# arnab39/equiadapt

Hardware: AMD Instinct MI355X
Metric: canonicalize+invert images/sec (224x224 C8) (higher is better)
Workload: dtype f32 (resampling / FFT / accumulation in fp32; the network's channel contraction as 2xfp16 split of every fp32 operand (within one fp32 ulp), 3 exact products, fp32 accumulate -- closer to fp64 than the fp32 matrix instruction, see step_ms_by_gemm_form); 1 GPU; configs[1]: 224x224x3 synthetic, C8, GroupEquivariantImageCanonicalization + ESCNNEquivariantNetwork in e2cnn's LAYER SHAPES (32 fields x 8 = 256 ch, k5, 3 layers, crop 0.8, resize 96) with this repository's own filter-bank parameterisation (bilinear-rotated banks; e2cnn's steerable basis is not restated -- e2cnn-trained weights enter via load_exported_dense), forward, then invert_canonicalization; batch_per_gpu=256, global_batch=256, parallelism=dp1 (no collective in the forward path)

## Files before the change

equiadapt_amd/_lib.py:

```python
import ctypes
import os
import subprocess
import threading

_HERE = os.path.dirname(os.path.abspath(__file__))
ROOT = os.path.dirname(_HERE)
CSRC = os.path.join(_HERE, "csrc")
SO_PATH = os.environ.get("EQA_LIB") or os.path.join(CSRC, "libeqa_hip.so")
SOURCES = [os.path.join(CSRC, f) for f in ("group_action.hip", "crop_resize.hip", "nearest_action.hip", "pooling.hip", "batchnorm.hip", "winograd.hip", "lift_conv.hip", "lift_conv_wide.hip", "lift_wgrad.hip", "pointcloud.hip", "vnsmall_train.hip", "vnsmall_tail.hip", "fftconv.hip", "fft_filter.hip", "lift_fft.hip", "cgemm3m.hip", "cgemm3m_bf16.hip", "smallconv.hip", "planegemm.hip", "convnet_train.hip")]
HEADERS = [os.path.join(CSRC, "eqa_common.hpp"), os.path.join(CSRC, "vn_common.hpp"), os.path.join(CSRC, "fft48.inc"), os.path.join(CSRC, "fft_common.inc"), os.path.join(CSRC, "cgemm3m_common.inc")]
INCLUDE = os.path.join(ROOT, "include")

ABI_VERSION = 3

_c_f = ctypes.POINTER(ctypes.c_float)
_c_i = ctypes.POINTER(ctypes.c_int32)
_vp = ctypes.c_void_p
_int = ctypes.c_int

SIGNATURES = {
    "eqa_abi_version": (_int, []),
    "eqa_set_option": (_int, [_int, _int]),
    "eqa_get_option": (_int, [_int]),
    "eqa_fold_edge_pad_workspace_bytes": (ctypes.c_int64, [_int] * 4),
    "eqa_fold_edge_pad": (_int, [_vp, _vp, _vp, _int, _int, _int, _int, _vp]),
    "eqa_canon_transform_fwd": (_int, [_vp, _vp, _vp, _vp, _vp] + [_int] * 6 + [_vp]),
    "eqa_invert_action_fwd": (_int, [_vp, _vp, _vp, _vp, _vp, _vp] + [_int] * 6 + [_vp]),
    "eqa_group_action_pair": (_int, [_vp] * 4 + [_int, _int] + [_vp] * 5 + [_int, _int, _vp] + [_int] * 4 + [_vp]),
    "eqa_orbit_expand_fwd": (_int, [_vp, _vp, _vp, _vp] + [_int] * 5 + [_vp]),
    "eqa_group_action_fwd": (_int, [_vp, _vp, _vp, _vp, _vp, _vp] + [_int] * 12 + [_vp]),
    "eqa_group_action_fwd_hint": (_int, [_vp, _vp, _vp, _vp, _vp, _vp] + [_int] * 13 + [_vp]),
    "eqa_crop_resize_aa": (_int, [_vp] * 6 + [_int] * 9 + [_vp]),
    "eqa_mask_action_nearest": (_int, [_vp] * 5 + [_int] * 4 + [_vp]),
    "eqa_mask_action_nearest_planes": (_int, [_vp] * 5 + [_int] * 4 + [_vp]),
    "eqa_boxes_action": (_int, [_vp] * 5 + [_int, ctypes.c_float, _int, _vp]),
    "eqa_image_action_nearest": (_int, [_vp] * 5 + [_int] * 10 + [_vp]),
    "eqa_group_action_bwd_tiles": (_int, [_int, _int]),
    "eqa_group_action_bwd": (_int, [_vp] * 8 + [_int] * 12 + [_vp]),
    "eqa_group_action_bwd_theta": (_int, [_vp] * 8 + [_int] * 12 + [_vp]),
    "eqa_group_pool_workspace_bytes": (ctypes.c_int64, [_int] * 4),
    "eqa_group_pool_argmax": (_int, [_vp, _vp, _vp, _vp] + [_int] * 4 + [_vp]),
    "eqa_window_sums": (_int, [_vp, _vp, _vp, _int, _vp] + [_int] * 5 + [_vp]),
    "eqa_bn_partial_blocks": (ctypes.c_int64, [ctypes.c_int64]),
    "eqa_bn_stats_nhwc": (_int, [_vp, _vp, ctypes.c_int64, _int, _vp]),
    "eqa_bn_relu_dropout_nhwc": (_int, [_vp, _vp, _vp, _vp, ctypes.c_int64, _int, ctypes.c_float, ctypes.c_uint32, _vp]),
    "eqa_bn_bwd_reduce_nhwc": (_int, [_vp] * 5 + [ctypes.c_float, _vp, ctypes.c_int64, _int, _vp, _vp, ctypes.c_uint32, _vp]),
    "eqa_bn_bwd_apply_nhwc": (_int, [_vp] * 8 + [ctypes.c_float, _vp, ctypes.c_int64, _int, _vp, _vp, ctypes.c_uint32, _vp]),
# ... 264 lines not shown
```

equiadapt_amd/csrc/crop_resize.hip:

```cpp
#include "eqa_common.hpp"

namespace {

constexpr int kAaBand = 8;
#ifndef EQA_AA_WIDE_MIN_K
#define EQA_AA_WIDE_MIN_K 8
#endif
constexpr int kAaMaxK = 20;

__global__ __launch_bounds__(kThreads) void crop_resize_aa_kernel(const float* __restrict__ x, float* __restrict__ y,
                                                                 const float* __restrict__ wx, const int32_t* __restrict__ x0,
                                                                 const float* __restrict__ wy, const int32_t* __restrict__ y0,
                                                                 int H, int W, int OH, int OW, int K, int max_rows) {
  extern __shared__ __attribute__((aligned(16))) float aa_tmp[];
  const int plane = blockIdx.y;
  const int r0 = blockIdx.x * kAaBand, r1 = min(r0 + kAaBand, OH);
  const int ybeg = y0[r0];
  const int yend = min(y0[r1 - 1] + K, H);
  const int nrows = min(yend - ybeg, max_rows);
  const float* src = x + (size_t)plane * H * W;
  const int rows_par = kThreads / OW;
  if (rows_par >= 1) {
    const int ox = threadIdx.x % OW, rsub = threadIdx.x / OW;
    if (rsub < rows_par) {
      const int xs = x0[ox];
      float wv[EQA_AA_WIDE_MIN_K];
      int xo[EQA_AA_WIDE_MIN_K];
#pragma unroll
// ... 14 lines not shown
      }
    }
  } else {
    for (int idx = threadIdx.x; idx < nrows * OW; idx += kThreads) {
      const int ry = idx / OW, ox = idx - ry * OW;
      const float* row = src + (size_t)(ybeg + ry) * W;
      const int xs = x0[ox];
      float acc = 0.0f;
#pragma unroll
      for (int j = 0; j < EQA_AA_WIDE_MIN_K; ++j)
        if (j < K) acc += wx[ox * K + j] * row[min(xs + j, W - 1)];
      aa_tmp[ry * OW + ox] = acc;
    }
  }
  __syncthreads();
  float* dst = y + (size_t)plane * OH * OW;
  for (int idx = threadIdx.x; idx < (r1 - r0) * OW; idx += kThreads) {
    const int r = idx / OW, ox = idx - r * OW;
    const int oy = r0 + r;

    const int ys = y0[oy] - ybeg;
    float acc = 0.0f;
#pragma unroll
    for (int j = 0; j < EQA_AA_WIDE_MIN_K; ++j)
      if (j < K) acc += wy[oy * K + j] * aa_tmp[min(ys + j, nrows - 1) * OW + ox];
    dst[(size_t)oy * OW + ox] = acc;
  }
}


template <int K, int BAND, int NL>
__global__ __launch_bounds__(kThreads, (NL > 5 && K > 5) ? 2 : 4) void crop_resize_aa_staged_kernel(
    const float* __restrict__ x, float* __restrict__ y,
                                                                        const float* __restrict__ wx, const int32_t* __restrict__ x0,
                                                                        const float* __restrict__ wy, const int32_t* __restrict__ y0,
                                                                        int planes, int H, int W, int OH, int OW, int cap_rows,
                                                                        int xb, int xl) {
  extern __shared__ __attribute__((aligned(16))) float aa_tmp[];
  float* rows = aa_tmp;
  float* tmp = aa_tmp + (size_t)cap_rows * xl;
  float* tabw = tmp + (size_t)cap_rows * OW;
  int* taby = reinterpret_cast<int*>(tabw + BAND * K);
  const int r0 = blockIdx.y * BAND, r1 = min(r0 + BAND, OH);
  const int nband = r1 - r0;
  const int plane0 = (int)(blockIdx.z * kXcd + blockIdx.x), plane_step = (int)(gridDim.z * kXcd);
  const int rows_par = kThreads / OW;
  const int ox = rows_par >= 1 ? threadIdx.x % OW : 0, rsub = rows_par >= 1 ? threadIdx.x / OW : 0;
  const int xs_g = x0[ox];
  float wv[K];
  int xo[K];
#pragma unroll
  for (int j = 0; j < K; ++j) {
    wv[j] = wx[ox * K + j];
    xo[j] = min(xs_g - xb + j, xl - 1);
  }
  if ((int)threadIdx.x < nband * K) tabw[threadIdx.x] = wy[r0 * K + threadIdx.x];
  const int ybeg = y0[r0];
  if ((int)threadIdx.x < nband) taby[threadIdx.x] = y0[r0 + threadIdx.x] - ybeg;
  const int yend = min(y0[r1 - 1] + K, H);
  const int nrows = min(yend - ybeg, cap_rows);
  const int nq = xl >> 2;
  const int tq = threadIdx.x & 63, tr = threadIdx.x >> 6;
  const bool prefetch = nq <= 64 && nrows <= 4 * NL;
  const size_t plane_sz = (size_t)H * W;
  const float* src0 = x + (size_t)ybeg * W + xb;
  typedef float aa_f4 __attribute__((ext_vector_type(4)));
  aa_f4 v[NL];
#define EQA_AA_PF_LOAD(plane_)                                                                                          \
  do {                                                                                                                  \
    const float* src_ = src0 + (size_t)(plane_) * plane_sz;                                                             \
    _Pragma("unroll") for (int k = 0; k < NL; ++k)                                                           \
      v[k] = *reinterpret_cast<const aa_f4*>(src_ + (size_t)min(tr + 4 * k, nrows - 1) * W + 4 * min(tq, nq - 1));     \
  } while (0)
  __builtin_amdgcn_s_waitcnt(0x0070);
  if (prefetch && plane0 < planes) EQA_AA_PF_LOAD(plane0);
  for (int plane = plane0; plane < planes; plane += plane_step) {
    if (prefetch) {
      if (tq < nq) {
#pragma unroll
        for (int k = 0; k < NL; ++k)
          if (tr + 4 * k < nrows) *reinterpret_cast<aa_f4*>(rows + (tr + 4 * k) * xl + 4 * tq) = v[k];
      }
      if (plane + plane_step < planes) EQA_AA_PF_LOAD(plane + plane_step);
    } else {
      const float* src = src0 + (size_t)plane * plane_sz;
      for (int q = tq; q < nq; q += 64)
        for (int rb = tr; rb < nrows; rb += 4) *reinterpret_cast<aa_f4*>(rows + rb * xl + 4 * q) = *reinterpret_cast<const aa_f4*>(src + (size_t)rb * W + 4 * q);
    }
    __syncthreads();
    if (rows_par >= 1) {
      if (rsub < rows_par) {
        for (int ry0 = rsub; ry0 < nrows; ry0 += 4 * rows_par) {
          float acc[4] = {0.0f, 0.0f, 0.0f, 0.0f};
#pragma unroll
          for (int u = 0; u < 4; ++u) {
            const float* row = rows + min(ry0 + u * rows_par, nrows - 1) * xl;
#pragma unroll
            for (int j = 0; j < K; ++j)
// ... 6 lines not shown
      }
    } else {
      for (int idx = threadIdx.x; idx < nrows * OW; idx += kThreads) {
        const int ry = idx / OW, oxx = idx - ry * OW;
        const float* row = rows + ry * xl;
        const int xs = x0[oxx] - xb;
        float acc = 0.0f;
#pragma unroll
        for (int j = 0; j < K; ++j)
          acc += wx[oxx * K + j] * row[min(xs + j, xl - 1)];
        tmp[ry * OW + oxx] = acc;
      }
    }
    __syncthreads();
    float* dst = y + (size_t)plane * OH * OW;
    for (int idx = threadIdx.x; idx < nband * OW; idx += kThreads) {
      const int r = idx / OW, oxx = idx - r * OW;
      const int ys = taby[r];
      float acc = 0.0f;
#pragma unroll
      for (int j = 0; j < K; ++j)
        acc += tabw[r * K + j] * tmp[min(ys + j, nrows - 1) * OW + oxx];
      dst[(size_t)(r0 + r) * OW + oxx] = acc;
    }
    __syncthreads();
  }
#undef EQA_AA_PF_LOAD
}

__global__ __launch_bounds__(kThreads) void crop_resize_aa_wide_kernel(const float* __restrict__ x, float* __restrict__ y,
                                                                      const float* __restrict__ wx, const int32_t* __restrict__ x0,
                                                                      const float* __restrict__ wy, const int32_t* __restrict__ y0,
                                                                      int H, int W, int OH, int OW, int K, int max_rows, int xbeg,
                                                                      int xlen, int pad_shift, int row_stride, int rpi) {
  extern __shared__ __attribute__((aligned(16))) float aa_tmp[];
  float* rowbuf = aa_tmp + (size_t)max_rows * OW;
  const int plane = blockIdx.y;
  const int r0 = blockIdx.x * kAaBand, r1 = min(r0 + kAaBand, OH);
  const int ybeg = y0[r0];
  const int yend = min(y0[r1 - 1] + K, H);
  const int nrows = min(yend - ybeg, max_rows);
  const float* src = x + (size_t)plane * H * W;
  auto pos = [&](int e) { return pad_shift ? e + (e >> pad_shift) : e; };
  const bool fixed_col = (kThreads % OW) == 0 && K <= kAaMaxK;
  const bool vec_stage = rpi <= 8 && (xlen & 3) == 0 && (xbeg & 3) == 0 && (W & 3) == 0 && ((((uintptr_t)src) & 15) == 0);
  const int ox_fixed = threadIdx.x % OW;
  const int xs_fixed = x0[ox_fixed] - xbeg;
  float wreg[kAaMaxK];
#pragma unroll
// ... 52 lines not shown
          if (j < K) acc += wreg[j] * row[pos(min(xs_fixed + j, xlen - 1))];
        aa_tmp[(ry0 + rr) * OW + ox_fixed] = acc;
      }
    } else {
      for (int idx = threadIdx.x; idx < nr * OW; idx += kThreads) {
        const int rr = idx / OW, ox = idx - rr * OW;
        const float* row = rowbuf + rr * row_stride;
        const int xs = x0[ox] - xbeg;
        float acc = 0.0f;
        for (int j = 0; j < K; ++j) acc += wx[ox * K + j] * row[pos(min(xs + j, xlen - 1))];
        aa_tmp[(ry0 + rr) * OW + ox] = acc;
      }
    }
    __syncthreads();
  }
  float* dst = y + (size_t)plane * OH * OW;
  for (int idx = threadIdx.x; idx < (r1 - r0) * OW; idx += kThreads) {
    const int r = idx / OW, ox = idx - r * OW;
    const int oy = r0 + r;
    const int ys = y0[oy] - ybeg;
    float acc = 0.0f;
    for (int j = 0; j < K; ++j) acc += wy[oy * K + j] * aa_tmp[min(ys + j, nrows - 1) * OW + ox];
    dst[(size_t)oy * OW + ox] = acc;
  }
}

constexpr int kAaStreamRows = 8;
__global__ __launch_bounds__(kThreads) void crop_resize_aa_stream_kernel(const float* __restrict__ x, float* __restrict__ y,
                                                                        const float* __restrict__ wx, const int32_t* __restrict__ x0,
                                                                        const float* __restrict__ wy, const int32_t* __restrict__ y0,
                                                                        int H, int W, int OH, int OW, int K, int xbeg, int xlen,
                                                                        int pad_shift, int row_stride) {
  extern __shared__ __attribute__((aligned(16))) float aa_rows[];
  const int plane = blockIdx.y;
  const int r0 = blockIdx.x * kAaBand, nr_out = min(kAaBand, OH - r0);
  int ys[kAaBand];
#pragma unroll
  for (int r = 0; r < kAaBand; ++r) ys[r] = y0[r0 + min(r, nr_out - 1)];
  const int ybeg = ys[0];
  const int span = ys[kAaBand - 1] + K - ybeg;
  const float* src = x + (size_t)plane * H * W + xbeg;
  const int e = 4 * (int)threadIdx.x;
  const int e_ld = min(e, xlen - 4);
  auto pos = [&](int i) { return pad_shift ? i + (i >> pad_shift) : i; };
  float4 acc[kAaBand];
#pragma unroll
  for (int r = 0; r < kAaBand; ++r) acc[r] = make_float4(0.f, 0.f, 0.f, 0.f);
// ... 19 lines not shown
        acc[r].x += w * v[q].x; acc[r].y += w * v[q].y; acc[r].z += w * v[q].z; acc[r].w += w * v[q].w;
      }
    }
  };
  static_assert(kAaStreamRows == 8 && kAaBand == 8, "one weight per lane: 8 rows of a trip x 8 output rows = 64 lanes");
  float4 va[kAaStreamRows], vb[kAaStreamRows];
  float wa, wb = 0.0f;
  load8(va, 0);
  wa = wload(0);
  for (int yc = 0; yc < span; yc += 2 * kAaStreamRows) {
    if (yc + kAaStreamRows < span) { load8(vb, yc + kAaStreamRows); wb = wload(yc + kAaStreamRows); }
    add8(va, wa);
    if (yc + 2 * kAaStreamRows < span) { load8(va, yc + 2 * kAaStreamRows); wa = wload(yc + 2 * kAaStreamRows); }
    if (yc + kAaStreamRows < span) add8(vb, wb);
  }
  float* dst = y + (size_t)plane * OH * OW;
#pragma unroll
  for (int half = 0; half < 2; ++half) {
    if (e < xlen) {
#pragma unroll
      for (int rr = 0; rr < kAaBand / 2; ++rr) {
        float* lrow = aa_rows + rr * row_stride;
        const float4 v = acc[half * (kAaBand / 2) + rr];
        lrow[pos(e)] = v.x; lrow[pos(e + 1)] = v.y; lrow[pos(e + 2)] = v.z; lrow[pos(e + 3)] = v.w;
      }
    }
    __syncthreads();
    for (int idx = threadIdx.x; idx < (kAaBand / 2) * OW; idx += kThreads) {
      const int rr = idx / OW, ox = idx - rr * OW;
      const int r = half * (kAaBand / 2) + rr;
      if (r < nr_out) {
        const float* row = aa_rows + rr * row_stride;
        const int xs = x0[ox] - xbeg;
        float a = 0.0f;
        for (int j = 0; j < K; ++j) a += wx[ox * K + j] * row[pos(min(xs + j, xlen - 1))];
        dst[(size_t)(r0 + r) * OW + ox] = a;
      }
    }
    __syncthreads();
  }
}

}

extern "C" {

int eqa_crop_resize_aa(const float* x, float* y, const float* wx, const int32_t* x0, const float* wy, const int32_t* y0,
                       int planes, int H, int W, int OH, int OW, int K, int max_rows, int x_begin, int x_span, void* stream) {
  if (!x || !y || !wx || !x0 || !wy || !y0 || planes < 0 || H <= 0 || W <= 0 || OH <= 0 || OW <= 0 || K <= 0 || max_rows <= 0)
    return EQA_ERR_INVALID_ARG;
  const size_t lds = (size_t)max_rows * OW * sizeof(float);
  if (lds > 96 * 1024 || planes > 65535) return EQA_ERR_UNSUPPORTED;
  if (planes == 0) return EQA_OK;
  const dim3 grid((OH + kAaBand - 1) / kAaBand, planes);
  if (K > EQA_AA_WIDE_MIN_K && x_span > 0 && x_begin >= 0 && x_begin + x_span <= W) {
    const int stride = (x_span + OW / 2) / OW;
    const int pad_shift = (stride >= 2 && (stride & 1) == 0) ? __builtin_ctz((unsigned)stride) : 0;
    const int row_stride = x_span + (pad_shift ? (x_span >> pad_shift) : 0) + 1;
    const size_t row_bytes = (size_t)row_stride * sizeof(float);
    const int rpi = (int)std::min<size_t>(8, lds + row_bytes <= 96 * 1024 ? (96 * 1024 - lds) / row_bytes : 0);
    const size_t lds2 = lds + (size_t)rpi * row_bytes;
    static const bool stream_off = [] { const char* e = getenv("EQA_AA_STREAM"); return e && e[0] == '0'; }();
    if (!stream_off && x_span <= 4 * kThreads && (x_span & 3) == 0 && (x_begin & 3) == 0 && (W & 3) == 0 && (((uintptr_t)x) & 15) == 0 &&
        (size_t)(kAaBand / 2) * row_bytes <= 64 * 1024) {
      hipLaunchKernelGGL(crop_resize_aa_stream_kernel, grid, dim3(kThreads), (kAaBand / 2) * row_bytes, (hipStream_t)stream, x, y, wx, x0, wy,
                         y0, H, W, OH, OW, K, x_begin, x_span, pad_shift, row_stride);
      return launch_status();
    }
    if (rpi >= 1) {
      hipLaunchKernelGGL(crop_resize_aa_wide_kernel, grid, dim3(kThreads), lds2, (hipStream_t)stream, x, y, wx, x0, wy, y0, H, W, OH,
                         OW, K, max_rows, x_begin, x_span, pad_shift, row_stride, rpi);
      return launch_status();
    }
  }
  static const bool staged_off = [] { const char* e = getenv("EQA_AA_STAGED"); return e && e[0] == '0'; }();
  if (!staged_off && K <= EQA_AA_WIDE_MIN_K && (W & 3) == 0 && (((uintptr_t)x) & 15) == 0 && x_span > 0 && x_begin >= 0 &&
      x_begin + x_span <= W) {
    const int xb = x_begin & ~3, xl = std::min(W, (x_begin + x_span + 3) & ~3) - xb;
    static const int band_env = [] { const char* e = getenv("EQA_AA_BAND"); return e ? atoi(e) : 0; }();
    int band = band_env == 16 ? 16 : (band_env == 8 ? 8 : (OH >= 64 ? 16 : 8));
    auto staged_lds = [&](int bnd) { return ((size_t)(bnd / kAaBand) * max_rows * (xl + OW) + bnd * (EQA_AA_WIDE_MIN_K + 1)) * sizeof(float); };
    if (band == 16 && band_env != 16 && (staged_lds(16) > 64 * 1024 || 16 * K > kThreads)) band = 8;
    const int cap_rows = (band / kAaBand) * max_rows;
    const size_t lds3 = staged_lds(band);
    if (lds3 <= 64 * 1024 && band * K <= kThreads) {
      static const int per_cu = [] { const char* e = getenv("EQA_AA_BLOCKS_PER_CU"); return e ? std::max(1, atoi(e)) : 12; }();
      const int nbands = (OH + band - 1) / band;
      const int groups = std::max(1, (std::min(planes, (256 * per_cu + nbands - 1) / nbands) + kXcd - 1) / kXcd);
      const bool few = cap_rows <= 20;
#define EQA_AA_STAGED(K_)                                                                                                              \
  case K_:                                                                                                                             \
    if (band == 16)                                                                                                                    \
      hipLaunchKernelGGL((crop_resize_aa_staged_kernel<K_, 16, 10>), dim3(kXcd, nbands, groups), dim3(kThreads), lds3, (hipStream_t)stream, x, \
                         y, wx, x0, wy, y0, planes, H, W, OH, OW, cap_rows, xb, xl);                                                   \
    else if (few)                                                                                                                      \
      hipLaunchKernelGGL((crop_resize_aa_staged_kernel<K_, 8, 5>), dim3(kXcd, nbands, groups), dim3(kThreads), lds3, (hipStream_t)stream, x,  \
                         y, wx, x0, wy, y0, planes, H, W, OH, OW, cap_rows, xb, xl);                                                   \
    else                                                                                                                               \
      hipLaunchKernelGGL((crop_resize_aa_staged_kernel<K_, 8, 10>), dim3(kXcd, nbands, groups), dim3(kThreads), lds3, (hipStream_t)stream, x, \
                         y, wx, x0, wy, y0, planes, H, W, OH, OW, cap_rows, xb, xl);                                                   \
    break
      switch (K) {
        EQA_AA_STAGED(1); EQA_AA_STAGED(2); EQA_AA_STAGED(3); EQA_AA_STAGED(4); EQA_AA_STAGED(5); EQA_AA_STAGED(6); EQA_AA_STAGED(7);
        EQA_AA_STAGED(8);
        default: return EQA_ERR_UNSUPPORTED;
      }
#undef EQA_AA_STAGED
      return launch_status();
    }
  }
  hipLaunchKernelGGL(crop_resize_aa_kernel, grid, dim3(kThreads), lds, (hipStream_t)stream, x, y, wx, x0, wy, y0, H, W, OH, OW, K,
                     max_rows);
  return launch_status();
}

}
```

equiadapt_amd/images/canonicalization/discrete_group.py:

```python
import math
from typing import Any, Dict, List, Optional, Tuple, Union

import torch
import torch.nn.functional as F

from equiadapt_amd import ops
from equiadapt_amd.common.basecanonicalization import DiscreteGroupCanonicalization
from equiadapt_amd.images import geometry
from equiadapt_amd.images.transforms import CenterCrop, EdgePad, Resize
from equiadapt_amd.images.utils import (
    canonicalize_masks,
    device_tables,
    canonicalize_boxes,
    flip_boxes,
    flip_masks,
    get_action_on_image_features,
    rotate_boxes,
    rotate_masks,
)



def _get(hyperparams: Any, name: str):
    if isinstance(hyperparams, dict):
# ... 88 lines not shown
        raise NotImplementedError(
            "get_group_activations is not implemented for the DiscreteGroupImageCanonicalization class")

    def get_groupelement(self, x: torch.Tensor) -> Dict[str, torch.Tensor]:
        group_activations = self.get_group_activations(x)
        group_index = self.group_index(group_activations)
        element = self.groupactivations_to_groupelement(group_activations, group_index)
        if not hasattr(self, "canonicalization_info_dict"):
            self.canonicalization_info_dict = {}
        self.canonicalization_info_dict["group_index"] = element.pop("group_index")
        self.canonicalization_info_dict["argmax_index"] = group_index
        self.canonicalization_info_dict["group_element"] = element
        self.canonicalization_info_dict["group_activations"] = group_activations
        return element

    def transformations_before_canonicalization_network_forward(self, x: torch.Tensor) -> torch.Tensor:
        crop, resize = self.crop_canonization, self.resize_canonization
        if (x.is_cuda and x.dtype == torch.float32 and not (torch.is_grad_enabled() and x.requires_grad) and isinstance(resize, Resize)
                and resize.antialias):
            from equiadapt_amd.images.transforms import resized_output_size

            out_hw = resized_output_size(crop.size, resize.size)
            if tuple(out_hw) == tuple(x.shape[-2:]) == tuple(crop.size):
                return x
            key = (tuple(x.shape[-2:]), crop.size, out_hw, str(x.device))
            tabs = self._consts.get(key)
            if tabs is None:
                t = geometry.aa_resize_tables(tuple(x.shape[-2:]), crop.size, out_hw)
                tabs = tuple(v.to(x.device) if isinstance(v, torch.Tensor) else v for v in t)
                self._consts[key] = tabs
            return ops.crop_resize_aa(x, tabs, out_hw)
        return resize(crop(x))


    def canonicalize(self, x: torch.Tensor, targets: Optional[List] = None, **kwargs: Any
                     ) -> Union[torch.Tensor, Tuple[torch.Tensor, List]]:
        self.device = x.device
        element = self.get_groupelement(x)
        gidx = self.canonicalization_info_dict["group_index"]
        reflections = "reflection" in element
        H, W = x.shape[-2:]
        pad = self.pad_size
        theta, flags = device_tables("canonicalize", self.num_rotations, reflections, (H + 2 * pad, W + 2 * pad), x.device)
        x = _CanonTransformFn.apply(x, element["rotation"], element.get("reflection"), gidx, theta, flags, pad,
                                    self.num_rotations)

# ... 44 lines not shown

def _num_group(group_type: str, num_rotations: int) -> int:
    return num_rotations if group_type == "rotation" else 2 * num_rotations


class GroupEquivariantImageCanonicalization(DiscreteGroupImageCanonicalization):

    def __init__(self, canonicalization_network: torch.nn.Module, canonicalization_hyperparams: Any, in_shape: tuple):
        super().__init__(canonicalization_network, canonicalization_hyperparams, in_shape)
        self.group_type = canonicalization_network.group_type
        self.num_rotations = canonicalization_network.num_rotations
        self.num_group = _num_group(self.group_type, self.num_rotations)
        self.group_info_dict = {"num_rotations": self.num_rotations, "num_group": self.num_group}

    def get_group_activations(self, x: torch.Tensor) -> torch.Tensor:
        x = self.transformations_before_canonicalization_network_forward(x)
        return self.canonicalization_network(x)


class OptimizedGroupEquivariantImageCanonicalization(DiscreteGroupImageCanonicalization):

    def __init__(self, canonicalization_network: torch.nn.Module, canonicalization_hyperparams: Any, in_shape: tuple):
        super().__init__(canonicalization_network, canonicalization_hyperparams, in_shape)
        self.group_type = _get(canonicalization_hyperparams, "group_type")
        self.num_rotations = _get(canonicalization_hyperparams, "num_rotations")
        self.artifact_err_wt = _get(canonicalization_hyperparams, "artifact_err_wt")
        self.num_group = _num_group(self.group_type, self.num_rotations)
        self.out_vector_size = canonicalization_network.out_vector_size
        size = _get(canonicalization_hyperparams, "resize_shape")
        self.group_augment_size = int(size)
        gray = self.in_shape[0] == 1
# ... 48 lines not shown
```

equiadapt_amd/images/canonicalization_networks/escnn_networks.py:

```python
import os
from typing import List, Sequence

import torch
import torch.nn as nn
import torch.nn.functional as F

from equiadapt_amd.images.canonicalization_networks.custom_group_equivariant_layers import (
    RotationEquivariantConv,
    RotationEquivariantConvLift,
    RotoReflectionEquivariantConv,
    RotoReflectionEquivariantConvLift,
)
from equiadapt_amd import ops
from equiadapt_amd.common.utils import update_running_stats
from equiadapt_amd.images.canonicalization_networks import fftconv, winograd
from equiadapt_amd.images.canonicalization_networks.pooling import (
    WindowSumsFunction,
    conv_then_group_pool,
    group_pool,
    window_sums_to_activations,
)


class _InnerBatchNorm(nn.BatchNorm3d):
# ... 557 lines not shown
            act = act + 0.0 * torch.stack(hidden_bias).sum().double()
        return act.float()

    def _training_fast_path_ok(self, x: torch.Tensor) -> bool:
        if self._dense or not x.is_cuda or x.dtype != torch.float32 or os.environ.get("EQA_TRAIN_FAST", "1") == "0":
            return False
        if (self.out_channels * self.num_group_elements) % 4 != 0:
            return False
        convs = [m for m in self.eqv_network if hasattr(m, "expanded_weights")]
        if len(convs) < 2 or any(c.stride != 1 or c.padding != 0 for c in convs) or not convs[-1].supports_linear_tail():
            return False
        hw = x.shape[-2] - (self.kernel_size - 1) * (len(convs) - 1)
        k = convs[-1].kernel_size
        return hw >= 2 * k - 1 and x.shape[-1] - (self.kernel_size - 1) * (len(convs) - 1) >= 2 * k - 1 and hw * hw <= 12288

    def forward(self, x: torch.Tensor) -> torch.Tensor:
        if (self.training or torch.is_grad_enabled()) and self._training_fast_path_ok(x):
            return self._forward_training(x)
        if not self.training and not torch.is_grad_enabled() and x.is_cuda and x.dtype == torch.float32:
            convs, norms = self._layers()
            shrink = (self.kernel_size - 1) * (len(convs) - 1)
            oh, ow = x.shape[-2] - shrink, x.shape[-1] - shrink
            if (convs[-1].supports_linear_tail() and 0 < oh and 0 < ow and oh * ow <= 12288
                    and all(n.running_mean is not None and not n.training for n in norms)
                    and all(c.stride == 1 and c.padding == 0 and c.kernel_size == self.kernel_size for c in convs)):
                return self._forward_inference(x)
        if self._dense:
            convs, norms = self._dense
            for i, cv in enumerate(convs):
                x = cv(x)
                if i < len(norms):
                    x = F.relu(norms[i](x))
            fm = x.reshape(x.shape[0], self.out_channels, self.num_group_elements, x.shape[-2], x.shape[-1])
        else:
            fm = self.eqv_network(x)
        return group_pool(fm)
```

equiadapt_amd/images/canonicalization_networks/fftconv.py:

```python
import math
import os
from typing import Optional

import torch

from equiadapt_amd import _lib, ops
from equiadapt_amd.ops import _timed

N, NH, OUT = 48, 25, 44
F = N * (NH - 2) + 2 * NH
ENABLED = os.environ.get("EQA_CONV5_FFT", "1") != "0"
MIN_TILES = int(os.environ.get("EQA_FFT_MIN_TILES", "32"))
TRAIN_FORWARD = os.environ.get("EQA_FFT_TRAIN", "1") != "0"
GEMM = os.environ.get("EQA_FFT_GEMM", "3m")
GEMM_PIECES = os.environ.get("EQA_FFT_GEMM_PIECES", "auto")
AUTO_MIN_CIN = int(os.environ.get("EQA_FFT_GEMM_AUTO_MIN_CIN", "128"))
AUTO_MIN_CIN_H3 = int(os.environ.get("EQA_FFT_GEMM_AUTO_MIN_CIN_H3", "64"))
DCMAX_SLOTS = 256
LAST_FORM = None


def f16_form_takes(cin: int, cout: int) -> bool:
    return cout % 128 == 0 and cin % 32 == 0

# ... 179 lines not shown
    def pieces(self) -> torch.Tensor:
        if self._pieces is None:
            self._pieces = self.split_bf16(self.bank)
        return self._pieces

    def spectra_into(self, V: torch.Tensor, B, st: int) -> Optional[torch.Tensor]:
        lib = _lib.load()
        nimg, C, H, W = self.shape
        dims = (nimg, H + 4, W + 4, C, st)
        px, pV = self.x.data_ptr(), V.data_ptr()
        p_b = self.bias.data_ptr() if self.bias is not None else None
        want_dc = self.relu and isinstance(B, Spectra3M) and gemm_form(B.cin, B.cout, True) == "h3"
        vbound = None
        if LIFT_FFT_FORM == "h2" and px % 16 == 0:
            wh, w_scale = self.pieces_f16()
            xbound = torch.empty(DCMAX_SLOTS, dtype=torch.float32, device=self.device)
            _lib.check(lib.eqa_absmax_slots(px, self.x.numel(), xbound.data_ptr(), st), "eqa_absmax_slots")
            if want_dc:
                vbound = torch.empty(DCMAX_SLOTS, dtype=torch.float32, device=self.device)
            _lib.check(lib.eqa_lift5_fft48k5_input_f16x2(px, wh.data_ptr(), w_scale, xbound.data_ptr(), DCMAX_SLOTS, p_b, int(self.relu), pV,
                                                         vbound.data_ptr() if want_dc else None, *dims), "eqa_lift5_fft48k5_input_f16x2")
        elif LIFT_FFT_FORM == "bf16x3":
            _lib.check(lib.eqa_lift5_fft48k5_input_bf16x3(px, self.pieces().data_ptr(), p_b, int(self.relu), pV, *dims),
                       "eqa_lift5_fft48k5_input_bf16x3")
        elif want_dc:
            vbound = torch.empty(DCMAX_SLOTS, dtype=torch.float32, device=self.device)
            _lib.check(lib.eqa_lift5_fft48k5_input_dcmax(px, self.bank.data_ptr(), p_b, 1, pV, vbound.data_ptr(), *dims),
                       "eqa_lift5_fft48k5_input_dcmax")
        else:
            _lib.check(lib.eqa_lift5_fft48k5_input(px, self.bank.data_ptr(), p_b, int(self.relu), pV, *dims), "eqa_lift5_fft48k5_input")
        return vbound

    def materialize(self) -> torch.Tensor:
        return ops.lift_conv_nhwc(self.x, ops.pack_lift_weights(self.bank), self.bias, self.relu, 5, 5)

# ... 282 lines not shown
```

equiadapt_amd/ops.py:

```python
from typing import Optional, Tuple

import torch

from equiadapt_amd import _lib


MAX_WINDOW_K = 10


def _stream() -> int:
    return _raw_stream(_current_device())


try:
    _raw_stream, _current_device = torch._C._cuda_getCurrentRawStream, torch._C._cuda_getDevice
except AttributeError:
    def _raw_stream(_dev):
        return torch.cuda.current_stream().cuda_stream

    def _current_device():
        return 0


class KernelTimer:
# ... 342 lines not shown
    if pooling not in ("mean", "max"):
        raise ValueError(f"Pooling type {pooling} not supported")
    if three != 3 or params.numel() != (1310 if pooling == "mean" else 1751):
        raise ValueError("vnsmall_canonicalize expects x:(B,3,N) and 1310 (mean) / 1751 (max) packed parameters")
    vec = torch.empty((B, 3, 3), dtype=torch.float32, device=x.device)
    R = torch.empty((B, 3, 3), dtype=torch.float32, device=x.device)
    y = torch.empty_like(x)
    ws = torch.empty((max(lib.eqa_vnsmall_workspace_bytes(B, N), 4) // 4,), dtype=torch.float32, device=x.device)
    with torch.cuda.device(x.device), _timed("vnsmall_fwd"):
        st = lib.eqa_vnsmall_canonicalize(x.data_ptr(), params.data_ptr(), vec.data_ptr(), R.data_ptr(), y.data_ptr(), ws.data_ptr(),
                                          B, N, k, int(pooling == "max"), _stream())
    _lib.check(st, "eqa_vnsmall_canonicalize")
    return vec, R, y


def crop_resize_aa(x: torch.Tensor, tables, out_hw: Tuple[int, int]) -> torch.Tensor:
    lib = _lib.load()
    x = _need(x, "x")
    wx, x0, wy, y0, K, max_rows, x_begin, x_span = tables
    B, C, H, W = x.shape
    y = torch.empty((B, C, out_hw[0], out_hw[1]), dtype=torch.float32, device=x.device)
    with torch.cuda.device(x.device), _timed("crop_resize_aa"):
        st = lib.eqa_crop_resize_aa(x.data_ptr(), y.data_ptr(), wx.data_ptr(), x0.data_ptr(), wy.data_ptr(), y0.data_ptr(),
                                    B * C, H, W, out_hw[0], out_hw[1], K, max_rows, x_begin, x_span, _stream())
    _lib.check(st, "eqa_crop_resize_aa")
    return y


def mask_action_nearest(masks: torch.Tensor, eidx: torch.Tensor, rtheta: torch.Tensor, flags: Optional[torch.Tensor]) -> torch.Tensor:
    lib = _lib.load()
    masks = _need(masks, "masks", torch.uint8)
    eidx = _need(eidx, "eidx", torch.int32)
    rtheta = _need(rtheta, "rtheta")
    flags, p_flags = _opt(flags, "flags", torch.int32)
    n, H, W = masks.shape
# ... 489 lines not shown
```

include/eqa_hip.h:

```cpp
#ifndef EQA_HIP_H
#define EQA_HIP_H

#include <stdint.h>

#ifdef __cplusplus
extern "C" {
#endif

#define EQA_OK 0
#define EQA_ERR_INVALID_ARG (-1)
#define EQA_ERR_LAUNCH (-2)
#define EQA_ERR_UNSUPPORTED (-3)

#define EQA_FLIP_SRC 1
#define EQA_FLIP_DST 2

#define EQA_ABI_VERSION 3
int eqa_abi_version(void);

int eqa_set_option(int key, int value);
int eqa_get_option(int key);

int eqa_canon_transform_fwd(const float* x, float* y, const int32_t* gidx, const float* theta,
                            const int32_t* flags, int num_elements, int B, int C, int H, int W, int pad,
// ... 8 lines not shown
                          const int32_t* chan_map, int G, int Cf, const int32_t* gidx, int num_elements, int B, int H,
                          int W, void* stream);

int eqa_orbit_expand_fwd(const float* x, float* y, const float* theta, const int32_t* flags, int num_elements,
                         int B, int C, int S, int pad, void* stream);

int eqa_group_action_fwd(const float* src, float* dst, const int32_t* gidx, const float* theta,
                         const int32_t* flags, const int32_t* chan_map, int num_elements, int G, int n_out,
                         int B, int C, int H, int W, int pad, int OH, int OW, int top, int left, void* stream);
int eqa_group_action_fwd_hint(const float* src, float* dst, const int32_t* gidx, const float* theta, const int32_t* flags,
                              const int32_t* chan_map, int num_elements, int G, int n_out, int B, int C, int H, int W,
                              int pad, int OH, int OW, int top, int left, int max_window, void* stream);

int eqa_crop_resize_aa(const float* x, float* y, const float* wx, const int32_t* x0, const float* wy, const int32_t* y0,
                       int planes, int H, int W, int OH, int OW, int K, int max_rows, int x_begin, int x_span, void* stream);

int eqa_mask_action_nearest(const uint8_t* m, uint8_t* out, const int32_t* eidx, const float* rtheta, const int32_t* flags,
                            int num_elements, int n_masks, int H, int W, void* stream);
int eqa_mask_action_nearest_planes(const uint8_t* const* planes, uint8_t* out, const int32_t* eidx, const float* rtheta,
                                   const int32_t* flags, int num_elements, int n_masks, int H, int W, void* stream);

int eqa_boxes_action(const float* boxes, const int32_t* img_of_box, const float* rotation_deg, float* flipped, float* out,
                     int n, float width, int flip_all, void* stream);

int eqa_image_action_nearest(const float* x, float* out, const int32_t* eidx, const float* rtheta, const int32_t* flags,
                             int num_elements, int n_planes, int src_mod, int H, int W, int pad, int OH, int OW, int top,
                             int left, void* stream);

int64_t eqa_fold_edge_pad_workspace_bytes(int planes, int H, int W, int pad);
int eqa_fold_edge_pad(const float* gframe, float* gsrc, void* workspace, int planes, int H, int W, int pad, void* stream);
// ... 228 lines not shown
```

Measured before the change: 70590 images/s.

## Emit channels-last crop-resize output with fused absmax bound for lift FFT

The anti-aliased crop-resize kernel can now write NHWC output directly, walking all channels of an image inside one block and interleaving them through LDS. It also computes a per-block absmax on the fly and hands it to the lift FFT stage, which would otherwise run a separate absmax pass over the same tensor. The network advertises when it wants channels-last input. The cost is extra LDS use and a slot buffer, plus a Python-side cache keyed on storage pointer and tensor version.

```diff
diff --git a/equiadapt_amd/_lib.py b/equiadapt_amd/_lib.py
--- a/equiadapt_amd/_lib.py
+++ b/equiadapt_amd/_lib.py
@@ -31,6 +31,8 @@
     "eqa_group_action_fwd": (_int, [_vp, _vp, _vp, _vp, _vp, _vp] + [_int] * 12 + [_vp]),
     "eqa_group_action_fwd_hint": (_int, [_vp, _vp, _vp, _vp, _vp, _vp] + [_int] * 13 + [_vp]),
     "eqa_crop_resize_aa": (_int, [_vp] * 6 + [_int] * 9 + [_vp]),
+    "eqa_crop_resize_aa_nhwc": (_int, [_vp] * 7 + [_int] * 10 + [_vp]),
+    "eqa_crop_resize_aa_nhwc_slots": (_int, [_vp] + [_int] * 10),
     "eqa_mask_action_nearest": (_int, [_vp] * 5 + [_int] * 4 + [_vp]),
     "eqa_mask_action_nearest_planes": (_int, [_vp] * 5 + [_int] * 4 + [_vp]),
     "eqa_boxes_action": (_int, [_vp] * 5 + [_int, ctypes.c_float, _int, _vp]),
diff --git a/equiadapt_amd/csrc/crop_resize.hip b/equiadapt_amd/csrc/crop_resize.hip
--- a/equiadapt_amd/csrc/crop_resize.hip
+++ b/equiadapt_amd/csrc/crop_resize.hip
@@ -8,10 +8,20 @@
 #endif
 constexpr int kAaMaxK = 20;
 
+struct AaOut {
+  float* p;
+  int ps;
+};
+__device__ __forceinline__ AaOut aa_out(float* y, int plane, int OH, int OW, int chan) {
+  if (chan <= 1) return {y + (size_t)plane * OH * OW, 1};
+  const int img = plane / chan;
+  return {y + (size_t)img * OH * OW * chan + (plane - img * chan), chan};
+}
+
 __global__ __launch_bounds__(kThreads) void crop_resize_aa_kernel(const float* __restrict__ x, float* __restrict__ y,
                                                                  const float* __restrict__ wx, const int32_t* __restrict__ x0,
                                                                  const float* __restrict__ wy, const int32_t* __restrict__ y0,
-                                                                 int H, int W, int OH, int OW, int K, int max_rows) {
+                                                                 int H, int W, int OH, int OW, int K, int max_rows, int chan) {
   extern __shared__ __attribute__((aligned(16))) float aa_tmp[];
   const int plane = blockIdx.y;
   const int r0 = blockIdx.x * kAaBand, r1 = min(r0 + kAaBand, OH);
@@ -56,7 +66,7 @@
     }
   }
   __syncthreads();
-  float* dst = y + (size_t)plane * OH * OW;
+  const AaOut dst = aa_out(y, plane, OH, OW, chan);
   for (int idx = threadIdx.x; idx < (r1 - r0) * OW; idx += kThreads) {
     const int r = idx / OW, ox = idx - r * OW;
     const int oy = r0 + r;
@@ -66,26 +76,29 @@
 #pragma unroll
     for (int j = 0; j < EQA_AA_WIDE_MIN_K; ++j)
       if (j < K) acc += wy[oy * K + j] * aa_tmp[min(ys + j, nrows - 1) * OW + ox];
-    dst[(size_t)oy * OW + ox] = acc;
-  }
-}
-
-
-template <int K, int BAND, int NL>
+    dst.p[((size_t)oy * OW + ox) * dst.ps] = acc;
+  }
+}
+
+
+struct alignas(4) AaPixel3 { float c[3]; };
+template <int K, int BAND, int NL, bool CL = false>
 __global__ __launch_bounds__(kThreads, (NL > 5 && K > 5) ? 2 : 4) void crop_resize_aa_staged_kernel(
     const float* __restrict__ x, float* __restrict__ y,
                                                                         const float* __restrict__ wx, const int32_t* __restrict__ x0,
                                                                         const float* __restrict__ wy, const int32_t* __restrict__ y0,
                                                                         int planes, int H, int W, int OH, int OW, int cap_rows,
-                                                                        int xb, int xl) {
+                                                                        int xb, int xl, int chan, float* __restrict__ absmax) {
   extern __shared__ __attribute__((aligned(16))) float aa_tmp[];
   float* rows = aa_tmp;
   float* tmp = aa_tmp + (size_t)cap_rows * xl;
   float* tabw = tmp + (size_t)cap_rows * OW;
   int* taby = reinterpret_cast<int*>(tabw + BAND * K);
+  float* keep = reinterpret_cast<float*>(taby + BAND);
   const int r0 = blockIdx.y * BAND, r1 = min(r0 + BAND, OH);
   const int nband = r1 - r0;
-  const int plane0 = (int)(blockIdx.z * kXcd + blockIdx.x), plane_step = (int)(gridDim.z * kXcd);
+  const int plane0 = (int)(blockIdx.z * kXcd + blockIdx.x) * (CL ? chan : 1), plane_step = (int)(gridDim.z * kXcd);
+  int cl_c = 0;
   const int rows_par = kThreads / OW;
   const int ox = rows_par >= 1 ? threadIdx.x % OW : 0, rsub = rows_par >= 1 ? threadIdx.x / OW : 0;
   const int xs_g = x0[ox];
@@ -108,6 +121,7 @@
   const float* src0 = x + (size_t)ybeg * W + xb;
   typedef float aa_f4 __attribute__((ext_vector_type(4)));
   aa_f4 v[NL];
+  float vmax = 0.0f;
 #define EQA_AA_PF_LOAD(plane_)                                                                                          \
   do {                                                                                                                  \
     const float* src_ = src0 + (size_t)(plane_) * plane_sz;                                                             \
@@ -116,14 +130,19 @@
   } while (0)
   __builtin_amdgcn_s_waitcnt(0x0070);
   if (prefetch && plane0 < planes) EQA_AA_PF_LOAD(plane0);
-  for (int plane = plane0; plane < planes; plane += plane_step) {
+  for (int plane = plane0, next; plane < planes; plane = next) {
+    if constexpr (CL) {
+      next = cl_c + 1 < chan ? plane + 1 : plane + 1 + (plane_step - 1) * chan;
+    } else {
+      next = plane + plane_step;
+    }
     if (prefetch) {
       if (tq < nq) {
 #pragma unroll
         for (int k = 0; k < NL; ++k)
           if (tr + 4 * k < nrows) *reinterpret_cast<aa_f4*>(rows + (tr + 4 * k) * xl + 4 * tq) = v[k];
       }
-      if (plane + plane_step < planes) EQA_AA_PF_LOAD(plane + plane_step);
+      if (next < planes) EQA_AA_PF_LOAD(next);
     } else {
       const float* src = src0 + (size_t)plane * plane_sz;
       for (int q = tq; q < nq; q += 64)
@@ -160,6 +179,7 @@
     }
     __syncthreads();
     float* dst = y + (size_t)plane * OH * OW;
+    if constexpr (CL) dst = y + (size_t)(plane - cl_c) * OH * OW;
     for (int idx = threadIdx.x; idx < nband * OW; idx += kThreads) {
       const int r = idx / OW, oxx = idx - r * OW;
       const int ys = taby[r];
@@ -167,18 +187,45 @@
 #pragma unroll
       for (int j = 0; j < K; ++j)
         acc += tabw[r * K + j] * tmp[min(ys + j, nrows - 1) * OW + oxx];
-      dst[(size_t)(r0 + r) * OW + oxx] = acc;
-    }
+      if constexpr (CL) {
+        vmax = fmaxf(vmax, fabsf(acc));
+        if (cl_c + 1 < chan) {
+          keep[cl_c * (BAND * OW) + idx] = acc;
+        } else {
+          float* px = dst + ((size_t)(r0 + r) * OW + oxx) * chan;
+          if (chan == 3) {
+            *reinterpret_cast<AaPixel3*>(px) = AaPixel3{{keep[idx], keep[BAND * OW + idx], acc}};
+          } else {
+            for (int c = 0; c + 1 < chan; ++c) px[c] = keep[c * (BAND * OW) + idx];
+            px[chan - 1] = acc;
+          }
+        }
+      } else {
+        dst[(size_t)(r0 + r) * OW + oxx] = acc;
+      }
+    }
+    if constexpr (CL) cl_c = cl_c + 1 < chan ? cl_c + 1 : 0;
     __syncthreads();
   }
 #undef EQA_AA_PF_LOAD
+  if constexpr (CL) {
+    if (absmax) {
+      __shared__ float red[kThreads / 64];
+#pragma unroll
+      for (int o = 32; o > 0; o >>= 1) vmax = fmaxf(vmax, __shfl_xor(vmax, o));
+      if ((threadIdx.x & 63) == 0) red[threadIdx.x >> 6] = vmax;
+      __syncthreads();
+      if (threadIdx.x == 0)
+        absmax[(blockIdx.z * gridDim.y + blockIdx.y) * gridDim.x + blockIdx.x] = fmaxf(fmaxf(red[0], red[1]), fmaxf(red[2], red[3]));
+    }
+  }
 }
 
 __global__ __launch_bounds__(kThreads) void crop_resize_aa_wide_kernel(const float* __restrict__ x, float* __restrict__ y,
                                                                       const float* __restrict__ wx, const int32_t* __restrict__ x0,
                                                                       const float* __restrict__ wy, const int32_t* __restrict__ y0,
                                                                       int H, int W, int OH, int OW, int K, int max_rows, int xbeg,
-                                                                      int xlen, int pad_shift, int row_stride, int rpi) {
+                                                                      int xlen, int pad_shift, int row_stride, int rpi, int chan) {
   extern __shared__ __attribute__((aligned(16))) float aa_tmp[];
   float* rowbuf = aa_tmp + (size_t)max_rows * OW;
   const int plane = blockIdx.y;
@@ -261,14 +308,14 @@
     }
     __syncthreads();
   }
-  float* dst = y + (size_t)plane * OH * OW;
+  const AaOut dst = aa_out(y, plane, OH, OW, chan);
   for (int idx = threadIdx.x; idx < (r1 - r0) * OW; idx += kThreads) {
     const int r = idx / OW, ox = idx - r * OW;
     const int oy = r0 + r;
     const int ys = y0[oy] - ybeg;
     float acc = 0.0f;
     for (int j = 0; j < K; ++j) acc += wy[oy * K + j] * aa_tmp[min(ys + j, nrows - 1) * OW + ox];
-    dst[(size_t)oy * OW + ox] = acc;
+    dst.p[((size_t)oy * OW + ox) * dst.ps] = acc;
   }
 }
 
@@ -277,7 +324,7 @@
                                                                         const float* __restrict__ wx, const int32_t* __restrict__ x0,
                                                                         const float* __restrict__ wy, const int32_t* __restrict__ y0,
                                                                         int H, int W, int OH, int OW, int K, int xbeg, int xlen,
-                                                                        int pad_shift, int row_stride) {
+                                                                        int pad_shift, int row_stride, int chan) {
   extern __shared__ __attribute__((aligned(16))) float aa_rows[];
   const int plane = blockIdx.y;
   const int r0 = blockIdx.x * kAaBand, nr_out = min(kAaBand, OH - r0);
@@ -327,7 +374,7 @@
     if (yc + 2 * kAaStreamRows < span) { load8(va, yc + 2 * kAaStreamRows); wa = wload(yc + 2 * kAaStreamRows); }
     if (yc + kAaStreamRows < span) add8(vb, wb);
   }
-  float* dst = y + (size_t)plane * OH * OW;
+  const AaOut dst = aa_out(y, plane, OH, OW, chan);
 #pragma unroll
   for (int half = 0; half < 2; ++half) {
     if (e < xlen) {
@@ -347,24 +394,25 @@
         const int xs = x0[ox] - xbeg;
         float a = 0.0f;
         for (int j = 0; j < K; ++j) a += wx[ox * K + j] * row[pos(min(xs + j, xlen - 1))];
-        dst[(size_t)(r0 + r) * OW + ox] = a;
-      }
-    }
-    __syncthreads();
-  }
-}
-
-}
-
-extern "C" {
-
-int eqa_crop_resize_aa(const float* x, float* y, const float* wx, const int32_t* x0, const float* wy, const int32_t* y0,
-                       int planes, int H, int W, int OH, int OW, int K, int max_rows, int x_begin, int x_span, void* stream) {
-  if (!x || !y || !wx || !x0 || !wy || !y0 || planes < 0 || H <= 0 || W <= 0 || OH <= 0 || OW <= 0 || K <= 0 || max_rows <= 0)
+        dst.p[((size_t)(r0 + r) * OW + ox) * dst.ps] = a;
+      }
+    }
+    __syncthreads();
+  }
+}
+
+}
+
+static int aa_launch(const float* x, float* y, const float* wx, const int32_t* x0, const float* wy, const int32_t* y0, int planes, int H,
+                     int W, int OH, int OW, int K, int max_rows, int x_begin, int x_span, int chan, float* absmax, int* nslots,
+                     void* stream) {
+  const bool query = nslots != nullptr;
+  if (query) *nslots = 0;
+  if (!x || (!query && (!y || !wx || !x0 || !wy || !y0)) || planes < 0 || H <= 0 || W <= 0 || OH <= 0 || OW <= 0 || K <= 0 || max_rows <= 0)
     return EQA_ERR_INVALID_ARG;
   const size_t lds = (size_t)max_rows * OW * sizeof(float);
   if (lds > 96 * 1024 || planes > 65535) return EQA_ERR_UNSUPPORTED;
-  if (planes == 0) return EQA_OK;
+  if (planes == 0) return absmax ? EQA_ERR_UNSUPPORTED : EQA_OK;
   const dim3 grid((OH + kAaBand - 1) / kAaBand, planes);
   if (K > EQA_AA_WIDE_MIN_K && x_span > 0 && x_begin >= 0 && x_begin + x_span <= W) {
     const int stride = (x_span + OW / 2) / OW;
@@ -376,13 +424,17 @@
     static const bool stream_off = [] { const char* e = getenv("EQA_AA_STREAM"); return e && e[0] == '0'; }();
     if (!stream_off && x_span <= 4 * kThreads && (x_span & 3) == 0 && (x_begin & 3) == 0 && (W & 3) == 0 && (((uintptr_t)x) & 15) == 0 &&
         (size_t)(kAaBand / 2) * row_bytes <= 64 * 1024) {
+      if (query) return EQA_OK;
+      if (absmax) return EQA_ERR_UNSUPPORTED;
       hipLaunchKernelGGL(crop_resize_aa_stream_kernel, grid, dim3(kThreads), (kAaBand / 2) * row_bytes, (hipStream_t)stream, x, y, wx, x0, wy,
-                         y0, H, W, OH, OW, K, x_begin, x_span, pad_shift, row_stride);
+                         y0, H, W, OH, OW, K, x_begin, x_span, pad_shift, row_stride, chan);
       return launch_status();
     }
     if (rpi >= 1) {
+      if (query) return EQA_OK;
+      if (absmax) return EQA_ERR_UNSUPPORTED;
       hipLaunchKernelGGL(crop_resize_aa_wide_kernel, grid, dim3(kThreads), lds2, (hipStream_t)stream, x, y, wx, x0, wy, y0, H, W, OH,
-                         OW, K, max_rows, x_begin, x_span, pad_shift, row_stride, rpi);
+                         OW, K, max_rows, x_begin, x_span, pad_shift, row_stride, rpi, chan);
       return launch_status();
     }
   }
@@ -392,26 +444,36 @@
     const int xb = x_begin & ~3, xl = std::min(W, (x_begin + x_span + 3) & ~3) - xb;
     static const int band_env = [] { const char* e = getenv("EQA_AA_BAND"); return e ? atoi(e) : 0; }();
     int band = band_env == 16 ? 16 : (band_env == 8 ? 8 : (OH >= 64 ? 16 : 8));
-    auto staged_lds = [&](int bnd) { return ((size_t)(bnd / kAaBand) * max_rows * (xl + OW) + bnd * (EQA_AA_WIDE_MIN_K + 1)) * sizeof(float); };
+    auto staged_lds = [&](int bnd) {
+      return ((size_t)(bnd / kAaBand) * max_rows * (xl + OW) + bnd * (EQA_AA_WIDE_MIN_K + 1) + (chan > 1 ? (size_t)(chan - 1) * bnd * OW : 0)) * sizeof(float);
+    };
     if (band == 16 && band_env != 16 && (staged_lds(16) > 64 * 1024 || 16 * K > kThreads)) band = 8;
     const int cap_rows = (band / kAaBand) * max_rows;
     const size_t lds3 = staged_lds(band);
     if (lds3 <= 64 * 1024 && band * K <= kThreads) {
       static const int per_cu = [] { const char* e = getenv("EQA_AA_BLOCKS_PER_CU"); return e ? std::max(1, atoi(e)) : 12; }();
       const int nbands = (OH + band - 1) / band;
-      const int groups = std::max(1, (std::min(planes, (256 * per_cu + nbands - 1) / nbands) + kXcd - 1) / kXcd);
+      const int units = chan > 1 ? planes / chan : planes;
+      const int groups = std::max(1, (std::min(units, (256 * per_cu + nbands - 1) / nbands) + kXcd - 1) / kXcd);
       const bool few = cap_rows <= 20;
+      if (query) {
+        *nslots = kXcd * nbands * groups;
+        return EQA_OK;
+      }
+      const dim3 sgrid(kXcd, nbands, groups);
+#define EQA_AA_STAGED_LAUNCH(K_, BAND_, NL_, CL_)                                                                                      \
+  hipLaunchKernelGGL((crop_resize_aa_staged_kernel<K_, BAND_, NL_, CL_>), sgrid, dim3(kThreads), lds3, (hipStream_t)stream, x, y, wx, x0, \
+                     wy, y0, planes, H, W, OH, OW, cap_rows, xb, xl, chan, absmax)
+#define EQA_AA_STAGED_FORM(K_, CL_)                                                                                                    \
+  do {                                                                                                                                 \
+    if (band == 16) EQA_AA_STAGED_LAUNCH(K_, 16, 10, CL_);                                                                             \
+    else if (few) EQA_AA_STAGED_LAUNCH(K_, 8, 5, CL_);                                                                                 \
+    else EQA_AA_STAGED_LAUNCH(K_, 8, 10, CL_);                                                                                         \
+  } while (0)
 #define EQA_AA_STAGED(K_)                                                                                                              \
   case K_:                                                                                                                             \
-    if (band == 16)                                                                                                                    \
-      hipLaunchKernelGGL((crop_resize_aa_staged_kernel<K_, 16, 10>), dim3(kXcd, nbands, groups), dim3(kThreads), lds3, (hipStream_t)stream, x, \
-                         y, wx, x0, wy, y0, planes, H, W, OH, OW, cap_rows, xb, xl);                                                   \
-    else if (few)                                                                                                                      \
-      hipLaunchKernelGGL((crop_resize_aa_staged_kernel<K_, 8, 5>), dim3(kXcd, nbands, groups), dim3(kThreads), lds3, (hipStream_t)stream, x,  \
-                         y, wx, x0, wy, y0, planes, H, W, OH, OW, cap_rows, xb, xl);                                                   \
-    else                                                                                                                               \
-      hipLaunchKernelGGL((crop_resize_aa_staged_kernel<K_, 8, 10>), dim3(kXcd, nbands, groups), dim3(kThreads), lds3, (hipStream_t)stream, x, \
-                         y, wx, x0, wy, y0, planes, H, W, OH, OW, cap_rows, xb, xl);                                                   \
+    if (chan > 1) EQA_AA_STAGED_FORM(K_, true);                                                                                        \
+    else EQA_AA_STAGED_FORM(K_, false);                                                                                                \
     break
       switch (K) {
         EQA_AA_STAGED(1); EQA_AA_STAGED(2); EQA_AA_STAGED(3); EQA_AA_STAGED(4); EQA_AA_STAGED(5); EQA_AA_STAGED(6); EQA_AA_STAGED(7);
@@ -419,12 +481,41 @@
         default: return EQA_ERR_UNSUPPORTED;
       }
 #undef EQA_AA_STAGED
+#undef EQA_AA_STAGED_FORM
+#undef EQA_AA_STAGED_LAUNCH
       return launch_status();
     }
   }
+  if (query) return EQA_OK;
+  if (absmax) return EQA_ERR_UNSUPPORTED;
   hipLaunchKernelGGL(crop_resize_aa_kernel, grid, dim3(kThreads), lds, (hipStream_t)stream, x, y, wx, x0, wy, y0, H, W, OH, OW, K,
-                     max_rows);
+                     max_rows, chan);
   return launch_status();
 }
 
-}
+extern "C" {
+
+int eqa_crop_resize_aa(const float* x, float* y, const float* wx, const int32_t* x0, const float* wy, const int32_t* y0,
+                       int planes, int H, int W, int OH, int OW, int K, int max_rows, int x_begin, int x_span, void* stream) {
+  return aa_launch(x, y, wx, x0, wy, y0, planes, H, W, OH, OW, K, max_rows, x_begin, x_span, 1, nullptr, nullptr, stream);
+}
+
+int eqa_crop_resize_aa_nhwc(const float* x, float* y, float* absmax, const float* wx, const int32_t* x0, const float* wy,
+                            const int32_t* y0, int nimg, int C, int H, int W, int OH, int OW, int K, int max_rows, int x_begin,
+                            int x_span, void* stream) {
+  if (nimg < 0 || C <= 0 || (int64_t)nimg * C > 0x7fffffffLL) return EQA_ERR_INVALID_ARG;
+  if (absmax && C <= 1) return EQA_ERR_UNSUPPORTED;
+  return aa_launch(x, y, wx, x0, wy, y0, nimg * C, H, W, OH, OW, K, max_rows, x_begin, x_span, C, absmax, nullptr, stream);
+}
+
+int eqa_crop_resize_aa_nhwc_slots(const float* x, int nimg, int C, int H, int W, int OH, int OW, int K, int max_rows, int x_begin,
+                                  int x_span) {
+  int n = 0;
+  if (nimg <= 0 || C <= 1 || (int64_t)nimg * C > 0x7fffffffLL) return 0;
+  if (aa_launch(x, nullptr, nullptr, nullptr, nullptr, nullptr, nimg * C, H, W, OH, OW, K, max_rows, x_begin, x_span, C, nullptr, &n,
+                nullptr) != EQA_OK)
+    return 0;
+  return n;
+}
+
+}
diff --git a/equiadapt_amd/images/canonicalization/discrete_group.py b/equiadapt_amd/images/canonicalization/discrete_group.py
--- a/equiadapt_amd/images/canonicalization/discrete_group.py
+++ b/equiadapt_amd/images/canonicalization/discrete_group.py
@@ -1,4 +1,5 @@
 import math
+import os
 from typing import Any, Dict, List, Optional, Tuple, Union
 
 import torch
@@ -126,7 +127,7 @@
         self.canonicalization_info_dict["group_activations"] = group_activations
         return element
 
-    def transformations_before_canonicalization_network_forward(self, x: torch.Tensor) -> torch.Tensor:
+    def transformations_before_canonicalization_network_forward(self, x: torch.Tensor, network=None) -> torch.Tensor:
         crop, resize = self.crop_canonization, self.resize_canonization
         if (x.is_cuda and x.dtype == torch.float32 and not (torch.is_grad_enabled() and x.requires_grad) and isinstance(resize, Resize)
                 and resize.antialias):
@@ -141,7 +142,9 @@
                 t = geometry.aa_resize_tables(tuple(x.shape[-2:]), crop.size, out_hw)
                 tabs = tuple(v.to(x.device) if isinstance(v, torch.Tensor) else v for v in t)
                 self._consts[key] = tabs
-            return ops.crop_resize_aa(x, tabs, out_hw)
+            asks = getattr(network, "channels_last_input", None)
+            cl = bool(asks((x.shape[0], x.shape[1], *out_hw))) if callable(asks) and os.environ.get("EQA_AA_NHWC", "1") != "0" else False
+            return ops.crop_resize_aa(x, tabs, out_hw, channels_last=cl, want_bound=cl)
         return resize(crop(x))
 
 
@@ -216,7 +219,7 @@
         self.group_info_dict = {"num_rotations": self.num_rotations, "num_group": self.num_group}
 
     def get_group_activations(self, x: torch.Tensor) -> torch.Tensor:
-        x = self.transformations_before_canonicalization_network_forward(x)
+        x = self.transformations_before_canonicalization_network_forward(x, network=self.canonicalization_network)
         return self.canonicalization_network(x)
 
 
diff --git a/equiadapt_amd/images/canonicalization_networks/escnn_networks.py b/equiadapt_amd/images/canonicalization_networks/escnn_networks.py
--- a/equiadapt_amd/images/canonicalization_networks/escnn_networks.py
+++ b/equiadapt_amd/images/canonicalization_networks/escnn_networks.py
@@ -595,17 +595,24 @@
         k = convs[-1].kernel_size
         return hw >= 2 * k - 1 and x.shape[-1] - (self.kernel_size - 1) * (len(convs) - 1) >= 2 * k - 1 and hw * hw <= 12288
 
+    def _inference_path_ok(self, shape) -> bool:
+        if self.training or torch.is_grad_enabled():
+            return False
+        convs, norms = self._layers()
+        shrink = (self.kernel_size - 1) * (len(convs) - 1)
+        oh, ow = shape[-2] - shrink, shape[-1] - shrink
+        return (convs[-1].supports_linear_tail() and 0 < oh and 0 < ow and oh * ow <= 12288
+                and all(n.running_mean is not None and not n.training for n in norms)
+                and all(c.stride == 1 and c.padding == 0 and c.kernel_size == self.kernel_size for c in convs))
+
+    def channels_last_input(self, shape) -> bool:
+        return (self.out_channels * self.num_group_elements) % 4 == 0 and self._inference_path_ok(shape)
+
     def forward(self, x: torch.Tensor) -> torch.Tensor:
         if (self.training or torch.is_grad_enabled()) and self._training_fast_path_ok(x):
             return self._forward_training(x)
-        if not self.training and not torch.is_grad_enabled() and x.is_cuda and x.dtype == torch.float32:
-            convs, norms = self._layers()
-            shrink = (self.kernel_size - 1) * (len(convs) - 1)
-            oh, ow = x.shape[-2] - shrink, x.shape[-1] - shrink
-            if (convs[-1].supports_linear_tail() and 0 < oh and 0 < ow and oh * ow <= 12288
-                    and all(n.running_mean is not None and not n.training for n in norms)
-                    and all(c.stride == 1 and c.padding == 0 and c.kernel_size == self.kernel_size for c in convs)):
-                return self._forward_inference(x)
+        if x.is_cuda and x.dtype == torch.float32 and self._inference_path_ok(x.shape):
+            return self._forward_inference(x)
         if self._dense:
             convs, norms = self._dense
             for i, cv in enumerate(convs):
diff --git a/equiadapt_amd/images/canonicalization_networks/fftconv.py b/equiadapt_amd/images/canonicalization_networks/fftconv.py
--- a/equiadapt_amd/images/canonicalization_networks/fftconv.py
+++ b/equiadapt_amd/images/canonicalization_networks/fftconv.py
@@ -217,11 +217,13 @@
         vbound = None
         if LIFT_FFT_FORM == "h2" and px % 16 == 0:
             wh, w_scale = self.pieces_f16()
-            xbound = torch.empty(DCMAX_SLOTS, dtype=torch.float32, device=self.device)
-            _lib.check(lib.eqa_absmax_slots(px, self.x.numel(), xbound.data_ptr(), st), "eqa_absmax_slots")
+            xbound = None if os.environ.get("EQA_HANDED_BOUND", "1") == "0" else ops.handed_bound(self.x)
+            if xbound is None:
+                xbound = torch.empty(DCMAX_SLOTS, dtype=torch.float32, device=self.device)
+                _lib.check(lib.eqa_absmax_slots(px, self.x.numel(), xbound.data_ptr(), st), "eqa_absmax_slots")
             if want_dc:
                 vbound = torch.empty(DCMAX_SLOTS, dtype=torch.float32, device=self.device)
-            _lib.check(lib.eqa_lift5_fft48k5_input_f16x2(px, wh.data_ptr(), w_scale, xbound.data_ptr(), DCMAX_SLOTS, p_b, int(self.relu), pV,
+            _lib.check(lib.eqa_lift5_fft48k5_input_f16x2(px, wh.data_ptr(), w_scale, xbound.data_ptr(), xbound.numel(), p_b, int(self.relu), pV,
                                                          vbound.data_ptr() if want_dc else None, *dims), "eqa_lift5_fft48k5_input_f16x2")
         elif LIFT_FFT_FORM == "bf16x3":
             _lib.check(lib.eqa_lift5_fft48k5_input_bf16x3(px, self.pieces().data_ptr(), p_b, int(self.relu), pV, *dims),
diff --git a/equiadapt_amd/ops.py b/equiadapt_amd/ops.py
--- a/equiadapt_amd/ops.py
+++ b/equiadapt_amd/ops.py
@@ -380,11 +380,61 @@
     return vec, R, y
 
 
-def crop_resize_aa(x: torch.Tensor, tables, out_hw: Tuple[int, int]) -> torch.Tensor:
+_handed_bounds: dict = {}
+
+
+def _bound_key(t: torch.Tensor):
+    return (t.device.index, t.untyped_storage().data_ptr())
+
+
+def _hand_bound(y: torch.Tensor, slots: torch.Tensor) -> None:
+    import weakref
+
+    try:
+        version = y._version
+    except RuntimeError:
+        return
+    key = _bound_key(y)
+    entry = (y.storage_offset(), y.numel(), version, slots)
+    _handed_bounds[key] = entry
+
+    def drop(key=key, entry=entry):
+        if _handed_bounds.get(key) is entry:
+            del _handed_bounds[key]
+
+    weakref.finalize(y.untyped_storage(), drop)
+
+
+def handed_bound(t: torch.Tensor) -> Optional[torch.Tensor]:
+    if not _handed_bounds or not t.is_cuda:
+        return None
+    hit = _handed_bounds.get(_bound_key(t))
+    if hit is None:
+        return None
+    try:
+        version = t._version
+    except RuntimeError:
+        return None
+    return hit[3] if (hit[0], hit[1], hit[2]) == (t.storage_offset(), t.numel(), version) else None
+
+
+def crop_resize_aa(x: torch.Tensor, tables, out_hw: Tuple[int, int], channels_last: bool = False, want_bound: bool = False) -> torch.Tensor:
     lib = _lib.load()
     x = _need(x, "x")
     wx, x0, wy, y0, K, max_rows, x_begin, x_span = tables
     B, C, H, W = x.shape
+    if channels_last and C > 1:
+        y = torch.empty((B, out_hw[0], out_hw[1], C), dtype=torch.float32, device=x.device).permute(0, 3, 1, 2)
+        shape = (B, C, H, W, out_hw[0], out_hw[1], K, max_rows, x_begin, x_span)
+        nslots = lib.eqa_crop_resize_aa_nhwc_slots(x.data_ptr(), *shape) if want_bound else 0
+        slots = torch.empty((nslots,), dtype=torch.float32, device=x.device) if nslots > 0 else None
+        with torch.cuda.device(x.device), _timed("crop_resize_aa"):
+            st = lib.eqa_crop_resize_aa_nhwc(x.data_ptr(), y.data_ptr(), slots.data_ptr() if slots is not None else None, wx.data_ptr(),
+                                             x0.data_ptr(), wy.data_ptr(), y0.data_ptr(), *shape, _stream())
+        _lib.check(st, "eqa_crop_resize_aa_nhwc")
+        if slots is not None:
+            _hand_bound(y, slots)
+        return y
     y = torch.empty((B, C, out_hw[0], out_hw[1]), dtype=torch.float32, device=x.device)
     with torch.cuda.device(x.device), _timed("crop_resize_aa"):
         st = lib.eqa_crop_resize_aa(x.data_ptr(), y.data_ptr(), wx.data_ptr(), x0.data_ptr(), wy.data_ptr(), y0.data_ptr(),
diff --git a/include/eqa_hip.h b/include/eqa_hip.h
--- a/include/eqa_hip.h
+++ b/include/eqa_hip.h
@@ -46,6 +46,11 @@
 
 int eqa_crop_resize_aa(const float* x, float* y, const float* wx, const int32_t* x0, const float* wy, const int32_t* y0,
                        int planes, int H, int W, int OH, int OW, int K, int max_rows, int x_begin, int x_span, void* stream);
+int eqa_crop_resize_aa_nhwc(const float* x, float* y, float* absmax, const float* wx, const int32_t* x0, const float* wy,
+                            const int32_t* y0, int nimg, int C, int H, int W, int OH, int OW, int K, int max_rows, int x_begin,
+                            int x_span, void* stream);
+int eqa_crop_resize_aa_nhwc_slots(const float* x, int nimg, int C, int H, int W, int OH, int OW, int K, int max_rows, int x_begin,
+                                  int x_span);
 
 int eqa_mask_action_nearest(const uint8_t* m, uint8_t* out, const int32_t* eidx, const float* rtheta, const int32_t* flags,
                             int num_elements, int n_masks, int H, int W, void* stream);
```

New measurement: 70870 images/s (median of 2 runs). Within noise of the previous version (+0.4%).
